# alpc91/SGRL

Hardware: AMD Instinct MI355X
Metric: env-steps/sec (whole node) + SET-actor fwd us/step, 3d_walker mix @8192 envs/GPU (higher is better)
Workload: dtype f64 (dynamics) / f32 (SET actor, obs); 1 GPU; 3D_Walker++ 8 variants x 1024 envs per GPU (config 3), random U(-1,1) actions, auto-reset, SET actor forward on every step, random-init weights; envs_per_gpu=8192, obs_max_len=287, action_max_len=21, replay_gather=none (single rank)

## Files before the change

include/sgrl.h:

```cpp
#ifndef SGRL_H
#define SGRL_H

#include <stdint.h>

#ifdef __cplusplus
extern "C" {
#endif

typedef struct sgrl_engine sgrl_engine;

enum {
  SGRL_OK = 0,
  SGRL_ERR_ARG = -1,
  SGRL_ERR_MODEL = -2,
  SGRL_ERR_HIP = -3,
  SGRL_ERR_LIMIT = -4
};

int sgrl_engine_create(int n_morph, const int32_t* const* ib, const int32_t* ib_len, const double* const* fb,
                       const int32_t* fb_len, const int32_t* morph_count, int obs_max_len, int action_max_len,
                       uint64_t seed, uint32_t env_id_base, int max_episode_steps, sgrl_engine** out);
void sgrl_engine_destroy(sgrl_engine* e);

int sgrl_num_envs(const sgrl_engine* e);
int sgrl_record_stride(const sgrl_engine* e);
int sgrl_lds_bytes(const sgrl_engine* e);
int sgrl_launch_groups(const sgrl_engine* e);
int sgrl_fixed_dim_groups(const sgrl_engine* e);
int sgrl_paired_envs(const sgrl_engine* e);

int sgrl_reset(sgrl_engine* e, float* obs, double* obs64, void* stream);

int sgrl_step(sgrl_engine* e, const float* actions, float* obs, float* reward, uint8_t* done, float* dist,
              uint8_t* truncated, double* obs64, double* reward64, int auto_reset, void* stream);

int sgrl_get_records(sgrl_engine* e, double* rec, int32_t* cnt);
int sgrl_set_records(sgrl_engine* e, const double* rec, const int32_t* cnt);
int sgrl_refresh(sgrl_engine* e, float* obs, double* obs64, void* stream);

int sgrl_time_steps(sgrl_engine* e, const float* actions, float* obs, float* reward, uint8_t* done, int reps,
                    void* stream, float* ms_out);

int sgrl_pack_transitions(const float* obs, int ld_obs, const float* action, int ld_act, const float* next_obs, int ld_next,
                          const float* reward, const float* done_f32, const uint8_t* done_u8, const uint8_t* store,
                          const int64_t* morph_id, float* block, int n_env, int obs_len, int act_len, void* stream);

int sgrl_round_record(const float* reward, const uint8_t* done, uint8_t* done_list, int64_t* ep_steps, float* ep_reward, float* reward_buf,
                      uint8_t* store, float* done_bool, int32_t* all_done, int n_env, int max_episode_steps, void* stream);

typedef struct sgrl_ring {
  float* obs; float* action; float* next_obs; float* reward; float* done;
  int32_t obs_dim, act_dim;
} sgrl_ring;
int sgrl_ingest_rows(const float* block, int n_rows, int obs_len, int act_len, const int64_t* slot, const sgrl_ring* rings,
                     int n_rings, void* stream);
int64_t sgrl_ingest_ws_words(int n_rows);
int sgrl_ingest_block(const float* block, int n_rows, int obs_len, int act_len, const sgrl_ring* rings, int n_rings, int64_t* pos,
                      const int64_t* cap, int64_t* pending, int64_t* slot_ws, void* stream);

const char* sgrl_last_error(void);
const char* sgrl_version(void);

#ifdef __cplusplus
}
#endif
#endif
```

sgrl_amd/_lib.py:

```python
import ctypes
import os
import subprocess

_HERE = os.path.dirname(os.path.abspath(__file__))
LIB_PATH = os.environ.get("SGRL_HIP_LIB", os.path.join(_HERE, "libsgrl_hip.so"))
CSRC = os.path.join(_HERE, "csrc")
SOURCES = ["engine.hip", "set_actor.hip", "train_gemm.hip", "render.hip", "swat_actor.hip", "smp_actor.hip", "replay_sample.hip", "eval_record.hip", "explore_actions.hip", "scene.hip", "mlp_actor.hip", "mlp_train.hip", "mlp_optim.hip", "mlp_batch.hip", "smp_train.hip", "td3_loss.hip", "dropout.hip"]

_lib = None

_i32p = ctypes.POINTER(ctypes.c_int32)
_f64p = ctypes.POINTER(ctypes.c_double)


class SgrlError(RuntimeError):
    pass


HDR_DIM_FIELDS = (1, 2, 3, 4, 5, 6, 7, 8, 9, 16, 18)
LIGHT_NV = 12
ITAB_GLOBAL = set(x for x in os.environ.get("SGRL_BUILD_ITAB_GLOBAL", "humanoid").split(",") if x and x != "none")
PAIR_NV = {"walker": 15, "hopper": 15}


# ... 96 lines not shown
    import torch
    try:
        L = ctypes.CDLL(LIB_PATH)
    except OSError as e:
        raise SgrlError("cannot load %s: %s" % (LIB_PATH, e))
    L.sgrl_last_error.restype = ctypes.c_char_p
    L.sgrl_version.restype = ctypes.c_char_p
    L.sgrl_engine_create.restype = ctypes.c_int
    L.sgrl_engine_create.argtypes = [ctypes.c_int, ctypes.POINTER(_i32p), _i32p, ctypes.POINTER(_f64p), _i32p, _i32p,
                                     ctypes.c_int, ctypes.c_int, ctypes.c_uint64, ctypes.c_uint32, ctypes.c_int,
                                     ctypes.POINTER(ctypes.c_void_p)]
    L.sgrl_engine_destroy.argtypes = [ctypes.c_void_p]
    L.sgrl_engine_destroy.restype = None
    for name in ("sgrl_num_envs", "sgrl_record_stride", "sgrl_lds_bytes", "sgrl_launch_groups", "sgrl_fixed_dim_groups", "sgrl_paired_envs"):
        getattr(L, name).argtypes = [ctypes.c_void_p]
        getattr(L, name).restype = ctypes.c_int
    vp = ctypes.c_void_p
    L.sgrl_reset.argtypes = [vp, vp, vp, vp]
    L.sgrl_step.argtypes = [vp, vp, vp, vp, vp, vp, vp, vp, vp, ctypes.c_int, vp]
    L.sgrl_refresh.argtypes = [vp, vp, vp, vp]
    L.sgrl_get_records.argtypes = [vp, vp, vp]
    L.sgrl_set_records.argtypes = [vp, vp, vp]
    L.sgrl_time_steps.argtypes = [vp, vp, vp, vp, vp, ctypes.c_int, vp, ctypes.POINTER(ctypes.c_float)]
    ci = ctypes.c_int
    L.sgrl_pack_transitions.argtypes = [vp, ci, vp, ci, vp, ci, vp, vp, vp, vp, vp, vp, ci, ci, ci, vp]
    L.sgrl_ingest_rows.argtypes = [vp, ci, ci, ci, vp, vp, ci, vp]
    L.sgrl_ingest_block.argtypes = [vp, ci, ci, ci, vp, ci, vp, vp, vp, vp, vp]
    L.sgrl_round_record.argtypes = [vp, vp, vp, vp, vp, vp, vp, vp, vp, ci, ci, vp]
    L.sgrl_ingest_ws_words.argtypes = [ci]
    L.sgrl_ingest_ws_words.restype = ctypes.c_int64
    _lib = L
    return L


EXPLORE_GAUSS, EXPLORE_UNIFORM = 0, 1


def bind_explore(L):
    if getattr(L, "_explore_bound", False):
        return L
    vp, ci, cf = ctypes.c_void_p, ctypes.c_int, ctypes.c_float
    L.sgrl_explore_actions.argtypes = [vp, ci, vp, ci, vp, ci, ci, ctypes.c_int64, ctypes.c_uint64, ctypes.c_uint64, ci, cf, cf, cf, vp]
    L.sgrl_explore_actions.restype = ci
    L.sgrl_explore_actions_launches.argtypes = []
    L.sgrl_explore_actions_launches.restype = ci
    L.sgrl_explore_last_error.argtypes = []
    L.sgrl_explore_last_error.restype = ctypes.c_char_p
    L._explore_bound = True
    return L


EXPORTS = ["sgrl_engine_create", "sgrl_engine_destroy", "sgrl_num_envs", "sgrl_record_stride", "sgrl_lds_bytes", "sgrl_launch_groups", "sgrl_fixed_dim_groups", "sgrl_paired_envs",
           "sgrl_reset", "sgrl_step", "sgrl_get_records", "sgrl_set_records", "sgrl_refresh", "sgrl_time_steps", "sgrl_pack_transitions", "sgrl_round_record", "sgrl_ingest_rows", "sgrl_ingest_block", "sgrl_ingest_ws_words",
           "sgrl_last_error", "sgrl_version"]


def check(rc, what):
    if rc != 0:
        raise SgrlError("%s failed (%d): %s" % (what, rc, lib().sgrl_last_error().decode()))
```

sgrl_amd/csrc/engine.hip:

```cpp
#include <hip/hip_runtime.h>

#include <algorithm>
#include <cmath>
#include <cstdio>
#include <cstdlib>
#include <cstring>
#include <string>
#include <vector>

#include "engine_kernel.h"
#include "stream_pick.h"

namespace {

thread_local std::string g_err;

int fail(int code, const std::string& msg) {
  g_err = msg;
  return code;
}
#define HIP_TRY(expr)                                                                              \
  do {                                                                                             \
    hipError_t _e = (expr);                                                                        \
    if (_e != hipSuccess)                                                                          \
      return fail(SGRL_ERR_HIP, std::string(#expr) + ": " + hipGetErrorString(_e));                \
  } while (0)

using namespace sgrl_engine_dev;

__global__ __launch_bounds__(64) __attribute__((amdgpu_waves_per_eu(2, 2))) void k_env_step(BatchArgs a, StepOut out) {
  env_step_wave<DimsAny, sgrl::HipWave>(a, out, __builtin_amdgcn_readfirstlane(a.block_env[blockIdx.x]));
}

constexpr int kLightNv = 15;
constexpr int kLightPerCu = 12;
__global__ __launch_bounds__(64) __attribute__((amdgpu_waves_per_eu(3, 3))) void k_env_step_light(BatchArgs a, StepOut out) {
  env_step_wave<DimsAny, sgrl::HipWaveT<kLightNv>>(a, out, __builtin_amdgcn_readfirstlane(a.block_env[blockIdx.x]));
}

__global__ __launch_bounds__(64) void k_env_reset(BatchArgs a, StepOut out) {
  const int env = __builtin_amdgcn_readfirstlane(a.block_env[blockIdx.x]);
  SgrlModelView m; sgrl::Layout o; double* S; int32_t* I;
  setup<DimsAny>(a, env, &m, &o, &S, &I);
  sgrl::HipWave w;
  const sgrl::StepIO io = make_io(a, out, env);
  sgrl::env_reset(w, m, o, S, I, io, true);
}

__global__ __launch_bounds__(64) void k_env_refresh(BatchArgs a, StepOut out) {
  const int env = __builtin_amdgcn_readfirstlane(a.block_env[blockIdx.x]);
  SgrlModelView m; sgrl::Layout o; double* S; int32_t* I;
  setup<DimsAny>(a, env, &m, &o, &S, &I);
  sgrl::HipWave w;
  const sgrl::StepIO io = make_io(a, out, env);
  sgrl::env_refresh(w, m, o, S, I, io);
}

typedef int (*SpecLaunch)(int, int, void*, const void*, const void*);
struct SpecFamily { int waves; int n; SpecLaunch launch; int itab_global; };
struct SpecMember { int family, slot; int dims[12]; };
}
#ifndef SGRL_NO_SPECS
#define SGRL_FAMILY(id, waves, n, itab) extern "C" int sgrl_spec_launch_##id(int, int, void*, const void*, const void*);
#define SGRL_MEMBER(...)
#include "spec_table.inc"
#undef SGRL_FAMILY
#undef SGRL_MEMBER
namespace {
const SpecFamily kFamilies[] = {
#define SGRL_FAMILY(id, waves, n, itab) {waves, n, sgrl_spec_launch_##id, itab},
#define SGRL_MEMBER(...)
#include "spec_table.inc"
#undef SGRL_FAMILY
#undef SGRL_MEMBER
};
const SpecMember kMembers[] = {
#define SGRL_FAMILY(id, waves, n, itab)
#define SGRL_MEMBER(fam, slot, ...) {fam, slot, {__VA_ARGS__}},
#include "spec_table.inc"
#undef SGRL_FAMILY
#undef SGRL_MEMBER
};
constexpr int kNumMembers = (int)(sizeof(kMembers) / sizeof(kMembers[0]));
}
#else
namespace {
const SpecFamily kFamilies[1] = {{0, 0, nullptr, 0}};
const SpecMember kMembers[1] = {{-1, -1, {0}}};
constexpr int kNumMembers = 0;
}
#endif
namespace {
int spec_for(const int32_t* hdr, int waves) {
  static const int fields[11] = {SGRL_H_NBODY, SGRL_H_NJNT, SGRL_H_NQ, SGRL_H_NV, SGRL_H_NU, SGRL_H_NGEOM, SGRL_H_NPAIR,
                                 SGRL_H_INTEGRATOR, SGRL_H_FRAME_SKIP, SGRL_H_MAX_ROWS, SGRL_H_SOLVER};
  for (int k = 0; k < kNumMembers; k++) {
    if (kFamilies[kMembers[k].family].waves != waves) continue;
    bool same = true;
    for (int f = 0; f < 11 && same; f++) same = kMembers[k].dims[f] == hdr[fields[f]];
    if (same) return k;
  }
  return -1;
}
}

struct sgrl_engine {
  int n_morph = 0, n_env = 0, stride = 0, lds_bytes = 0, scratch_stride = 0;
  int obs_max_len = 0, action_max_len = 0;
// ... 188 lines not shown
      for (int g = grp; g < (int)gridDim.x; g += kIngestThreads / kIngestMaxRings) p += w.chunk_hist[g * kIngestMaxRings + ring];
      part[grp][ring] = p;
    }
    __syncthreads();
    if (t < n_rings) {
      long long total = 0;
#pragma unroll
      for (int g = 0; g < kIngestThreads / kIngestMaxRings; g++) total += part[g][t];
      const long long p0 = pos[t];
      w.base[t] = p0;
      pos[t] = (p0 + total) % cap[t];
      pending[t] += total;
    }
    if (t == 0) *w.ticket = 0u;
  }
}
__global__ __launch_bounds__(kIngestThreads) void k_ingest_slots(int n_rows, const long long* __restrict__ cap, long long* ws, long long* __restrict__ slot) {
  __shared__ int keys[kIngestChunk];
  __shared__ int part[8][kIngestMaxRings];
  const IngestWs w = ingest_ws(ws, n_rows);
  const int t = threadIdx.x, c = blockIdx.x, r = c * kIngestChunk + t;
  const int k = r < n_rows ? w.key[r] : -1;
  keys[t] = k;
  {
    const int ring = t & 31, grp = t >> 5;
    int p = 0;
    for (int g = grp; g < c; g += 8) p += w.chunk_hist[g * kIngestMaxRings + ring];
    part[grp][ring] = p;
  }
  __syncthreads();
  long long sl = -1;
  if (k >= 0) {
    int rank = 0;
#pragma unroll
    for (int g = 0; g < 8; g++) rank += part[g][k];
    for (int j = 0; j < t; j++) rank += keys[j] == k ? 1 : 0;
    sl = (w.base[k] + rank) % cap[k];
  }
  if (r < n_rows) slot[r] = sl;
}

extern "C" {

const char* sgrl_last_error(void) { return g_err.c_str(); }
const char* sgrl_version(void) { return "sgrl-hip 0.2.0 (gfx950)"; }
#ifdef SGRL_PHASE_PROF
int sgrl_phase_prof(unsigned long long* host, int n_env, int reset) {
  if (hipDeviceSynchronize() != hipSuccess) return -1;
  if (host && hipMemcpyFromSymbol(host, HIP_SYMBOL(sgrl_engine_dev::g_phase_prof), sizeof(unsigned long long) * 16 * (size_t)n_env) != hipSuccess) return -2;
  if (reset) { static unsigned long long z[16 * 65536]; if (hipMemcpyToSymbol(HIP_SYMBOL(sgrl_engine_dev::g_phase_prof), z, sizeof(z)) != hipSuccess) return -3; }
  return 0;
}
#endif

void sgrl_engine_destroy(sgrl_engine* e) {
  if (!e) return;
  for (auto p : e->d_ib) if (p) (void)hipFree(p);
  for (auto p : e->d_fb) if (p) (void)hipFree(p);
  if (e->d_morphs) (void)hipFree(e->d_morphs);
  if (e->d_env_morph) (void)hipFree(e->d_env_morph);
  if (e->d_block_env) (void)hipFree(e->d_block_env);
  if (e->d_step_env) (void)hipFree(e->d_step_env);
  if (e->d_step_mate) (void)hipFree(e->d_step_mate);
  if (e->d_rec) (void)hipFree(e->d_rec);
  if (e->d_cnt) (void)hipFree(e->d_cnt);
  if (e->d_scratch) (void)hipFree(e->d_scratch);
  if (e->d_cam_dist) (void)hipFree(e->d_cam_dist);
  for (auto& g : e->groups) { if (g.stream) (void)hipStreamDestroy(g.stream); if (g.done) (void)hipEventDestroy(g.done); }
  if (e->fork) (void)hipEventDestroy(e->fork);
  delete e;
}

int sgrl_engine_create(int n_morph, const int32_t* const* ib, const int32_t* ib_len, const double* const* fb,
                       const int32_t* fb_len, const int32_t* morph_count, int obs_max_len, int action_max_len,
                       uint64_t seed, uint32_t env_id_base, int max_episode_steps, sgrl_engine** out) {
  if (!out) return fail(SGRL_ERR_ARG, "out is null");
  *out = nullptr;
  if (n_morph <= 0 || !ib || !ib_len || !fb || !fb_len || !morph_count) return fail(SGRL_ERR_ARG, "null or empty morphology list");
  int ndev = 0;
  (void)hipGetLastError();
  const hipError_t dev_err = hipGetDeviceCount(&ndev);
  if (dev_err != hipSuccess || ndev == 0)
    return fail(SGRL_ERR_HIP, std::string("no HIP device visible: libsgrl_hip.so needs an MI355X (there is no CPU fallback) [") +
                                  hipGetErrorString(dev_err) + ", " + std::to_string(ndev) + " devices]");
  sgrl_engine* e = new sgrl_engine();
  e->n_morph = n_morph;
  e->obs_max_len = obs_max_len;
  e->action_max_len = action_max_len;
  std::vector<int32_t> env_morph;
  std::vector<MorphDev> morphs(n_morph);
  e->d_ib.assign(n_morph, nullptr);
  e->d_fb.assign(n_morph, nullptr);
  int rc = SGRL_OK;
  for (int k = 0; k < n_morph && rc == SGRL_OK; k++) {
    SgrlModelView v;
    if (!ib[k] || !fb[k] || ib_len[k] < SGRL_NHDR || sgrl_model_view(ib[k], fb[k], &v) != 0) { rc = fail(SGRL_ERR_MODEL, "bad magic in model blob " + std::to_string(k)); break; }
    if (v.n_int != ib_len[k] || v.n_f64 != fb_len[k]) { rc = fail(SGRL_ERR_MODEL, "model blob " + std::to_string(k) + " has unexpected length"); break; }
    if (v.nv > 64 || v.nbody > 64 || v.npair > 64) { rc = fail(SGRL_ERR_LIMIT, "morphology exceeds 64 dofs/bodies/pairs"); break; }
    if ((v.nv | 1) > sgrl::kSlabLdy || ib[k][SGRL_H_MAX_ROWS] > sgrl::kSlabRows) { rc = fail(SGRL_ERR_LIMIT, "morphology exceeds the HBM constraint slab (nv <= 46, max_rows <= 256)"); break; }
    e->scratch_stride = std::max(e->scratch_stride, sgrl::slab_doubles(ib[k][SGRL_H_MAX_ROWS], v.nv | 1));
    e->max_geoms = std::max(e->max_geoms, v.ngeom);
    const int L = v.nbody - 1;
    if (41 * L > obs_max_len || 3 * L > action_max_len) { rc = fail(SGRL_ERR_ARG, "obs_max_len/action_max_len too small for morphology " + std::to_string(k)); break; }
    if (morph_count[k] < 0) { rc = fail(SGRL_ERR_ARG, "negative morph_count"); break; }
    sgrl::Layout o;
    sgrl::make_layout(ib[k], &o, v.n_int, SGRL_STAGE_FLOATS ? v.n_f64 : 0);
// ... 364 lines not shown
```

sgrl_amd/csrc/step_body.h:

```cpp
#pragma once

#include <math.h>
#include <stdint.h>

#include "../../include/sgrl_model.h"

#ifdef __HIPCC__
#define SGRL_DEV __device__ __forceinline__
#else
#define SGRL_DEV inline
#endif

namespace sgrl {

constexpr double kMinVal = 1e-15;
constexpr double kMinImp = 0.0001;
constexpr double kMaxImp = 0.9999;
constexpr double kPi = 3.14159265358979323846;
constexpr int kNAMax = 32;
constexpr int kBppMaxIter = 40;
constexpr int kSlabRows = 256;
constexpr int kPivotRows = 64;
constexpr int kPrevRows = 48;
constexpr int kSlabLdy = 47;
// ... 218 lines not shown
  double a[3], b[3], c[3];
  cross3(a, vel, f); cross3(b, vel + 3, f + 3); cross3(c, vel, f + 3);
  r[0] = a[0] + b[0]; r[1] = a[1] + b[1]; r[2] = a[2] + b[2];
  r[3] = c[0]; r[4] = c[1]; r[5] = c[2];
}
SGRL_DEV void ld3(double* r, const double* p) { r[0] = p[0]; r[1] = p[1]; r[2] = p[2]; }
SGRL_DEV void ld6(double* r, const double* p) { r[0] = p[0]; r[1] = p[1]; r[2] = p[2]; r[3] = p[3]; r[4] = p[4]; r[5] = p[5]; }
SGRL_DEV int popcount64(uint64_t x) {
#ifdef __HIPCC__
  return __popcll(x);
#else
  return __builtin_popcountll(x);
#endif
}
SGRL_DEV int clz64(uint64_t x) {
#ifdef __HIPCC__
  return __clzll((long long)x);
#else
  return __builtin_clzll(x);
#endif
}
SGRL_DEV int tri(int i) { return i * (i + 1) / 2; }
SGRL_DEV void tri_decode(int p, int* a_out, int* b_out) {
  int a = (int)((sqrtf(8.0f * (float)p + 1.0f) - 1.0f) * 0.5f);
  a += ((a + 1) * (a + 2) / 2 <= p) ? 1 : 0;
  a -= (a * (a + 1) / 2 > p) ? 1 : 0;
  *a_out = a; *b_out = p - a * (a + 1) / 2;
}
SGRL_DEV bool dof_in_mask(sgrl_itab_t mask2, int d) {
  const uint32_t w = (uint32_t)(d < 32 ? mask2[0] : mask2[1]);
  return (w >> (d & 31)) & 1u;
}

SGRL_DEV double rng_uniform01(uint64_t seed, uint32_t env_id, uint32_t episode, uint32_t stream, uint32_t idx) {
  uint32_t c0 = idx >> 2, c1 = episode, c2 = stream, c3 = (uint32_t)(seed >> 32);
  uint32_t k0 = (uint32_t)seed, k1 = env_id;
  for (int r = 0; r < 10; r++) {
    const uint64_t p0 = (uint64_t)0xD2511F53u * c0, p1 = (uint64_t)0xCD9E8D57u * c2;
    const uint32_t n0 = (uint32_t)(p1 >> 32) ^ c1 ^ k0, n1 = (uint32_t)p1;
    const uint32_t n2 = (uint32_t)(p0 >> 32) ^ c3 ^ k1, n3 = (uint32_t)p0;
    c0 = n0; c1 = n1; c2 = n2; c3 = n3;
    k0 += 0x9E3779B9u; k1 += 0xBB67AE85u;
  }
  const uint32_t lane = idx & 3u;
  const uint32_t x = lane == 0 ? c0 : (lane == 1 ? c1 : (lane == 2 ? c2 : c3));
  return ((double)x + 0.5) * (1.0 / 4294967296.0);
}

#ifdef SGRL_PHASE_PROF
#define SGRL_TICK(id) w.tick(id)
#else
#define SGRL_TICK(id)
#endif

template <class W>
struct Engine {
  W& w;
  SgrlModelView m;
  const Layout& o;
  double* S;
  int32_t* I;
  double* big_scratch = nullptr;
  bool linv = false;

  SGRL_DEV Engine(W& w_, const SgrlModelView& m_, const Layout& o_, double* S_, int32_t* I_)
      : w(w_), m(m_), o(o_), S(S_), I(I_) {}

  SGRL_DEV void fence_view() {
    if (W::kFixedDims) return;
    m.body_parent = w.fenced(m.body_parent); m.body_jntadr = w.fenced(m.body_jntadr);
    m.body_jntnum = w.fenced(m.body_jntnum); m.body_dofadr = w.fenced(m.body_dofadr);
    m.body_dofnum = w.fenced(m.body_dofnum); m.body_limbtype = w.fenced(m.body_limbtype);
    m.jnt_type = w.fenced(m.jnt_type); m.jnt_body = w.fenced(m.jnt_body);
    m.jnt_qposadr = w.fenced(m.jnt_qposadr); m.jnt_dofadr = w.fenced(m.jnt_dofadr);
    m.jnt_limited = w.fenced(m.jnt_limited); m.dof_body = w.fenced(m.dof_body); m.dof_jnt = w.fenced(m.dof_jnt);
    m.dof_parent = w.fenced(m.dof_parent); m.geom_type = w.fenced(m.geom_type);
    m.geom_body = w.fenced(m.geom_body); m.pair_g1 = w.fenced(m.pair_g1); m.pair_g2 = w.fenced(m.pair_g2);
    m.pair_condim = w.fenced(m.pair_condim); m.act_dof = w.fenced(m.act_dof); m.act_slot = w.fenced(m.act_slot);
    m.body_depth = w.fenced(m.body_depth); m.body_path = w.fenced(m.body_path);
    m.body_subend = w.fenced(m.body_subend); m.body_dofmask = w.fenced(m.body_dofmask);
    m.dof_act = w.fenced(m.dof_act);
  }

  SGRL_DEV static void quat_rot(double* r, const double* q, const double* v) {
    double mtx[9];
    quat2mat(mtx, q);
    mat_vec(r, mtx, v);
  }

  SGRL_DEV void kinematics() {
    w.lanes(1, [&](int) {
      double q[4] = {S[o.qpos + 3], S[o.qpos + 4], S[o.qpos + 5], S[o.qpos + 6]};
      quat_normalize(q);
      S[o.qpos + 3] = q[0]; S[o.qpos + 4] = q[1]; S[o.qpos + 5] = q[2]; S[o.qpos + 6] = q[3];
    });
    const int TJ = o.Y, TB = o.Y + 17 * o.nj;
    w.lanes(o.nj, [&](int j) {
      if (m.jnt_type[j] == SGRL_JNT_FREE) return;
      double ja[3], ql[4];
      ld3(ja, m.jnt_axis + 3 * j);
      const int qa = m.jnt_qposadr[j];
      axisangle2quat(ql, ja, S[o.qpos + qa] - m.qpos0[qa]);
      double* t = S + TJ + 17 * j;
      for (int k = 0; k < 4; k++) t[k] = ql[k];
      for (int k = 0; k < 3; k++) { t[4 + k] = ja[k]; t[7 + k] = m.jnt_pos[3 * j + k]; }
    });
// ... 574 lines not shown
        if (hk[r] == key) { f0 = hf[r]; hit = true; }
      }
      if (!hit) {
        for (int k = 0; k < pl; k++) if (I[o.prev_key + k] == key) f0 = S[o.prev_f + k];
        if (pn > pcap) {
          const double* hf = big_scratch + slab_prev_offset(o.maxrows, o.ldy);
          const int32_t* hk = reinterpret_cast<const int32_t*>(hf + o.maxrows);
          for (int k = pcap; k < pn; k++) if (hk[k] == key) f0 = hf[k];
        }
      }
      R.ef[r] = f0;
    });
    SGRL_TICK(6);
    if (linv) {
      if (BIG || !w.trmm_rows(nrow + 1, nv, S + o.L, R.Y, ldy))
      w.lanes(nrow + 1, [&](int r) {
        double* Yr = R.Y + r * ldy;
        for (int d = nv - 1; d >= 0; d--) {
          const double* Ld = S + o.L + tri(d);
          double s0 = 0, s1 = 0, s2 = 0, s3 = 0;
          int c = 0;
          for (; c + 4 <= d + 1; c += 4) {
            const double a0 = Ld[c], a1 = Ld[c + 1], a2 = Ld[c + 2], a3 = Ld[c + 3];
            const double b0 = Yr[c], b1 = Yr[c + 1], b2 = Yr[c + 2], b3 = Yr[c + 3];
            s0 += a0 * b0; s1 += a1 * b1; s2 += a2 * b2; s3 += a3 * b3;
          }
          for (; c <= d; c++) s0 += Ld[c] * Yr[c];
          Yr[d] = (s0 + s1) + (s2 + s3);
        }
      });
    } else {
      w.trsm_lower_rows(nrow + 1, nv, S + o.L, S + o.dinv, R.Y, ldy);
    }
    SGRL_TICK(9);
    w.lanes(nrow > nv ? nrow : nv, [&](int r) {
      if (r < nrow) {
        const double* Yr = R.Y + r * ldy;
        const double* ys = R.Y + nrow * ldy;
        double q0 = 0, q1 = 0, t0 = 0, t1 = 0;
        int d = 0;
        for (; d + 2 <= nv; d += 2) {
          const double y0 = Yr[d], y1 = Yr[d + 1];
          q0 += y0 * y0; q1 += y1 * y1; t0 += y0 * ys[d]; t1 += y1 * ys[d + 1];
        }
        for (; d < nv; d++) { q0 += Yr[d] * Yr[d]; t0 += Yr[d] * ys[d]; }
        const double Rr = R.eR[r];
        R.eidg[r] = 1.0 / ((q0 + q1) + Rr);
        R.eb[r] = (t0 + t1) - R.earef[r];
      }
      if (r < nv) S[o.vpgs + r] = 0;
    });
  }

  template <bool SMALL, bool CLDS>
  SGRL_DEV bool lcp_block_pivot(const Rows& R, int n, double thresh, int* iters_out) {
    double* const wvp = R.earef;
    double* const xwp = SMALL ? S + o.prev_f : S + o.Y;
    const int nv = o.nv, ldy = o.ldy;
    uint64_t F = w.ballot(n, [&](int i) { return R.ef[i] > 0.0; });
    int patience = 3, best = n + 1;
    for (int iter = 0; iter < kBppMaxIter; iter++) {
      w.fence_lane();
      const int nf = popcount64(F);
      double* const C = CLDS ? S + o.dead : R.C;
      w.lanes(n, [&](int i) {
        if ((F >> i) & 1ull) {
          const int pos = popcount64(F & ((1ull << i) - 1ull));
          R.flist[pos] = i;
          xwp[pos] = -R.eb[i];
        }
      });
      if (!w.aff_rows(nf, nv, R.Y, ldy, R.flist, R.eR, C))
      w.lanes(nf * (nf + 1) / 2, [&](int p) {
        int i, j;
        tri_decode(p, &i, &j);
        const int fi = R.flist[i], fj = R.flist[j];
        const double* yi = R.Y + fi * ldy;
        const double* yj = R.Y + fj * ldy;
        double s0 = 0, s1 = 0, s2 = 0, s3 = 0;
        int d = 0;
        for (; d + 4 <= nv; d += 4) {
          const double a0 = yi[d], a1 = yi[d + 1], a2 = yi[d + 2], a3 = yi[d + 3];
          const double b0 = yj[d], b1 = yj[d + 1], b2 = yj[d + 2], b3 = yj[d + 3];
          s0 += a0 * b0; s1 += a1 * b1; s2 += a2 * b2; s3 += a3 * b3;
        }
        for (; d < nv; d++) s0 += yi[d] * yj[d];
        double a = (s0 + s1) + (s2 + s3);
        if (i == j) a += R.eR[fi];
        C[p] = a;
      });
      SGRL_TICK(12);
      if (SMALL && w.chol_inv_packed(nf, C, kMinVal)) {
        w.lanes(nf, [&](int i) {
          double z = 0;
          for (int c = 0; c <= i; c++) z += C[i * (i + 1) / 2 + c] * xwp[c];
          wvp[i] = z;
        });
        w.lanes(nf, [&](int k) {
          double x = 0;
          for (int i = k; i < nf; i++) x += C[i * (i + 1) / 2 + k] * wvp[i];
          xwp[k] = x;
        });
      } else {
        for (int j = 0; j < nf - 1; j++) {
          double pj = C[j * (j + 1) / 2 + j];
          if (pj < kMinVal) pj = kMinVal;
          const double wj = 1.0 / pj;
          const int sdim = nf - j - 1;
          w.lanes(sdim * (sdim + 1) / 2, [&](int p) {
            int a, b;
            tri_decode(p, &a, &b);
            const int i = j + 1 + a, k = j + 1 + b;
            C[i * (i + 1) / 2 + k] -= C[i * (i + 1) / 2 + j] * C[k * (k + 1) / 2 + j] * wj;
          });
        }
        w.lanes(nf, [&](int j) {
          double pj = C[j * (j + 1) / 2 + j];
          if (pj < kMinVal) pj = kMinVal;
          wvp[j] = 1.0 / pj;
        });
        for (int j = 0; j < nf; j++) {
          const double zj = xwp[j] * wvp[j];
          w.lanes_from(j + 1, nf, [&](int i) { xwp[i] -= C[i * (i + 1) / 2 + j] * zj; });
        }
        w.lanes(nf, [&](int i) { xwp[i] *= wvp[i]; });
        for (int j = nf - 1; j > 0; j--) {
          const double xj = xwp[j];
          w.lanes(j, [&](int k) { xwp[k] -= C[j * (j + 1) / 2 + k] * wvp[k] * xj; });
        }
      }
      SGRL_TICK(13);
      w.lanes(nv, [&](int d) {
        double u0 = 0, u1 = 0;
        int k = 0;
        for (; k + 2 <= nf; k += 2) { u0 += R.Y[R.flist[k] * ldy + d] * xwp[k]; u1 += R.Y[R.flist[k + 1] * ldy + d] * xwp[k + 1]; }
        if (k < nf) u0 += R.Y[R.flist[k] * ldy + d] * xwp[k];
        S[o.vpgs + d] = u0 + u1;
      });
      const uint64_t V = w.ballot(n, [&](int i) {
        if ((F >> i) & 1ull) return xwp[popcount64(F & ((1ull << i) - 1ull))] < -thresh * R.eidg[i];
        const double* yi = R.Y + i * ldy;
        double y0 = R.eb[i], y1 = 0, y2 = 0, y3 = 0;
        int d = 0;
        for (; d + 4 <= nv; d += 4) {
          y0 += yi[d] * S[o.vpgs + d]; y1 += yi[d + 1] * S[o.vpgs + d + 1];
// ... 438 lines not shown
```

sgrl_amd/csrc/wave_half.h:

```cpp
#pragma once
#include <stdint.h>

#include "step_body.h"

namespace sgrl {

template <int NVCAP, class P>
struct HalfWaveT : P {
  static_assert(NVCAP <= 16, "the register solvers of a half wave keep one matrix row per lane of ONE 16-lane DPP row");
  using P::lane;
  static constexpr int kLanes = 32;

  template <class F> SGRL_DEV void lanes(int n, F f) {
    for (int i = lane; i < n; i += kLanes) f(i);
    P::sync();
  }
  template <class F> SGRL_DEV void lanes_from(int lo, int hi, F f) {
    for (int i = lo + lane; i < hi; i += kLanes) f(i);
    P::sync();
  }
  template <class F> SGRL_DEV double sum(int n, F f) {
    double p = 0.0;
    for (int i = lane; i < n; i += kLanes) p += f(i);
    return P::half_sum(p);
  }
  template <class F> SGRL_DEV double maxabs(int n, F f) {
    double p = 0.0;
    for (int i = lane; i < n; i += kLanes) p = fmax(p, fabs(f(i)));
    return P::half_max(p);
  }
  template <class F> SGRL_DEV uint64_t ballot(int n, F f) {
    uint64_t m = P::half_ballot(lane < n ? (bool)f(lane) : false);
    if (n > kLanes) m |= (uint64_t)P::half_ballot(lane + kLanes < n ? (bool)f(lane + kLanes) : false) << 32;
    return m;
  }

  template <int NMAX>
  SGRL_DEV void chol_inv_reg(int n, double* Pm, double minval) {
    const bool act = lane < n;
    const int li = act ? lane : 0;
    double* rowp = Pm + li * (li + 1) / 2;
    double a[NMAX + 1];
#pragma unroll
    for (int k = 0; k < NMAX; k++) a[k + 1] = rowp[k < li ? k : li];
    double mydj = 0.0;
#pragma unroll
    for (int j = 0; j < NMAX; j++) {
      if (j < n) {
        const double c = a[j + 1];
        double pj = P::bcast16(c, j);
        pj = pj < minval ? minval : pj;
        const double dj = inv_sqrt(pj);
        const double l = c * dj;
        mydj = lane == j ? dj : mydj;
        const double lm = lane > j ? l * dj : 0.0;
        a[j] = lane == j ? 1.0 : 0.0;
#pragma unroll
        for (int c2 = 0; c2 <= j; c2++) a[c2] -= lm * P::bcast16(a[c2], j);
#pragma unroll
        for (int k = j + 1; k < NMAX; k++) a[k + 1] -= l * P::bcast16(l, k);
      }
    }
    if (act) {
#pragma unroll
      for (int k = NMAX - 1; k >= 0; k--) rowp[k < li ? k : li] = a[k] * mydj;
    }
    P::sync();
  }
  SGRL_DEV bool chol_inv_packed(int n, double* Pm, double minval) {
    if (NVCAP >= 9 && n <= 9) chol_inv_reg<9>(n, Pm, minval);
    else if (NVCAP >= 12 && n <= 12) chol_inv_reg<12>(n, Pm, minval);
    else if (NVCAP >= 15 && n <= 15) chol_inv_reg<15>(n, Pm, minval);
    else return false;
    return true;
  }

  template <int NMAX>
  SGRL_DEV void trmm_rows_reg(int nrhs, int n, const double* T, double* Y, int ldy) {
    constexpr int NH = (NMAX + 1) / 2;
    const int h = lane & 1;
    for (int r0 = 0; r0 < nrhs; r0 += kLanes / 2) {
      const int r = r0 + (lane >> 1);
      const bool act = r < nrhs;
      double* y = Y + (act ? r : nrhs - 1) * ldy;
      double jr[NH];
#pragma unroll
      for (int u = 0; u < NH; u++) {
        const int c = 2 * u + h;
        const double v = y[c < n ? c : n - 1];
        jr[u] = c < n ? v : 0.0;
      }
#pragma unroll
      for (int d = (NMAX - 1) | 1; d >= 1; d -= 2) {
        if (d - 1 < n) {
          const double* Td = T + d * (d + 1) / 2 + h;
          const double* Te = T + (d - 1) * d / 2 + h;
          double s0 = 0.0, s1 = 0.0, e0 = 0.0, e1 = 0.0;
#pragma unroll
          for (int u = 0; u < NH; u++) {
            if (2 * u + 1 <= d) {
              const double td = Td[2 * u], te = Te[2 * u];
              const double tem = (2 * u + 1 <= d - 1) ? te : (h == 0 ? te : 0.0);
              if (u & 1) { s1 += td * jr[u]; e1 += tem * jr[u]; } else { s0 += td * jr[u]; e0 += tem * jr[u]; }
            }
          }
          double sd = s0 + s1, se = e0 + e1;
          sd += P::xor1(sd);
          se += P::xor1(se);
          if (act) { if (h == 0) y[d - 1] = se; else if (d < n) y[d] = sd; }
        }
      }
    }
    P::sync();
  }
  SGRL_DEV bool trmm_rows(int nrhs, int n, const double* T, double* Y, int ldy) {
#ifdef SGRL_NO_TRMM
    return false;
#endif
    if (NVCAP >= 9 && n <= 9) trmm_rows_reg<9>(nrhs, n, T, Y, ldy);
    else if (NVCAP >= 12 && n <= 12) trmm_rows_reg<12>(nrhs, n, T, Y, ldy);
    else if (NVCAP >= 15 && n <= 15) trmm_rows_reg<15>(nrhs, n, T, Y, ldy);
    else return false;
    return true;
  }
  SGRL_DEV bool aff_rows(int, int, const double*, int, const int32_t*, const double*, double*) { return false; }
// ... 68 lines not shown
```

sgrl_amd/csrc/wave_hip.h:

```cpp
#pragma once
#include <hip/hip_runtime.h>

#include "../../include/sgrl_model.h"

namespace sgrl {

template <int CTRL>
__device__ __forceinline__ double dpp_move(double x) {
  int lo = __double2loint(x), hi = __double2hiint(x);
  lo = __builtin_amdgcn_update_dpp(0, lo, CTRL, 0xF, 0xF, false);
  hi = __builtin_amdgcn_update_dpp(0, hi, CTRL, 0xF, 0xF, false);
  return __hiloint2double(hi, lo);
}
__device__ __forceinline__ double read_lane(double x, int l) {
  const int lo = __builtin_amdgcn_readlane(__double2loint(x), l);
  const int hi = __builtin_amdgcn_readlane(__double2hiint(x), l);
  return __hiloint2double(hi, lo);
}
__device__ __forceinline__ double wave_sum(double x) {
  x += dpp_move<0xB1>(x);
  x += dpp_move<0x4E>(x);
  x += dpp_move<0x141>(x);
  x += dpp_move<0x140>(x);
  return (read_lane(x, 0) + read_lane(x, 16)) + (read_lane(x, 32) + read_lane(x, 48));
// ... 138 lines not shown
        change = fmax(change, fabs(df) / ir);
      }
      __syncthreads();
      if (change < thresh) { it++; break; }
    }
    if (dofl) v[lane] = vv;
    __syncthreads();
    return it;
  }
  template <int NMAX>
  __device__ __forceinline__ void chol_inv_reg(int n, double* P, double minval) {
    const bool act = lane < n;
    const int li = act ? lane : 0;
    double* rowp = P + li * (li + 1) / 2;
    double a[NMAX + 1];
#pragma unroll
    for (int k = 0; k < NMAX; k++) a[k + 1] = rowp[k < li ? k : li];
    double mydj = 0.0;
#pragma unroll
    for (int j = 0; j < NMAX; j++) {
      if (j < n) {
        const double c = a[j + 1];
        double pj = read_lane(c, j);
        pj = pj < minval ? minval : pj;
        const double dj = rsqrt(pj);
        const double l = c * dj;
        mydj = lane == j ? dj : mydj;
        const double lm = lane > j ? l * dj : 0.0;
        a[j] = lane == j ? 1.0 : 0.0;
#pragma unroll
        for (int c2 = 0; c2 <= j; c2++) a[c2] -= lm * read_lane(a[c2], j);
#pragma unroll
        for (int k = j + 1; k < NMAX; k++) a[k + 1] -= l * read_lane(l, k);
      }
    }
    if (act) {
#pragma unroll
      for (int k = NMAX - 1; k >= 0; k--) rowp[k < li ? k : li] = a[k] * mydj;
    }
    __syncthreads();
  }
  __device__ __forceinline__ bool chol_inv_packed(int n_in, double* P, double minval) {
    const int n = __builtin_amdgcn_readfirstlane(n_in);
    if (NVCAP >= 9 && n <= 9) chol_inv_reg<9>(n, P, minval);
    else if (NVCAP >= 12 && n <= 12) chol_inv_reg<12>(n, P, minval);
    else if (NVCAP >= 15 && n <= 15) chol_inv_reg<15>(n, P, minval);
    else if (NVCAP >= 18 && n <= 18) chol_inv_reg<18>(n, P, minval);
    else if (NVCAP >= 21 && n <= 21) chol_inv_reg<21>(n, P, minval);
    else if (NVCAP >= 24 && n <= 24) chol_inv_reg<24>(n, P, minval);
    else return false;
    return true;
  }
  template <int NMAX>
  __device__ __forceinline__ void trmm_rows_reg(int nrhs, int n, const double* T, double* Y, int ldy) {
    constexpr int NH = (NMAX + 1) / 2;
    const int h = lane & 1;
    for (int r0 = 0; r0 < nrhs; r0 += 32) {
      const int r = r0 + (lane >> 1);
      const bool act = r < nrhs;
      double* y = Y + (act ? r : nrhs - 1) * ldy;
      double jr[NH];
#pragma unroll
      for (int u = 0; u < NH; u++) {
        const int c = 2 * u + h;
        const double v = y[c < n ? c : n - 1];
        jr[u] = c < n ? v : 0.0;
      }
#pragma unroll
      for (int d = (NMAX - 1) | 1; d >= 1; d -= 2) {
        if (d - 1 < n) {
          const double* Td = T + d * (d + 1) / 2 + h;
          const double* Te = T + (d - 1) * d / 2 + h;
          double s0 = 0.0, s1 = 0.0, e0 = 0.0, e1 = 0.0;
#pragma unroll
          for (int u = 0; u < NH; u++) {
            if (2 * u + 1 <= d) {
              const double td = Td[2 * u], te = Te[2 * u];
              const double tem = (2 * u + 1 <= d - 1) ? te : (h == 0 ? te : 0.0);
              if (u & 1) { s1 += td * jr[u]; e1 += tem * jr[u]; } else { s0 += td * jr[u]; e0 += tem * jr[u]; }
            }
          }
          double sd = s0 + s1, se = e0 + e1;
          sd += dpp_move<0xB1>(sd);
          se += dpp_move<0xB1>(se);
          if (act) { if (h == 0) y[d - 1] = se; else if (d < n) y[d] = sd; }
        }
      }
    }
    __syncthreads();
  }
  __device__ __forceinline__ void trmm_rows_mfma(int nrhs, int n, const double* T, double* Y, int ldy) {
    const int lo = lane & 15, hi = lane >> 4;
    const int ksteps = (n + 3) >> 2;
    for (int r0 = 0; r0 < nrhs; r0 += 16) {
      const int r = r0 + lo;
      const bool rv = r < nrhs;
      const double* yr = Y + (rv ? r : 0) * ldy;
      double b[6];
#pragma unroll
      for (int s = 0; s < 6; s++) {
        const int c = 4 * s + hi;
        const double v = yr[c < n ? c : 0];
        b[s] = (rv && c < n) ? v : 0.0;
      }
#pragma unroll
      for (int dt = 0; dt < 2; dt++) {
// ... 221 lines not shown
```

Measured before the change: 2.035 million env-steps/s.

## Fuse Cholesky factorization with forward/back solve instead of explicit inverse

Measured after the change: 2.079 million env-steps/s (median of 6 runs). 2.2% higher.

```diff
diff --git a/include/sgrl.h b/include/sgrl.h
--- a/include/sgrl.h
+++ b/include/sgrl.h
@@ -58,6 +58,9 @@
 int sgrl_ingest_block(const float* block, int n_rows, int obs_len, int act_len, const sgrl_ring* rings, int n_rings, int64_t* pos,
                       const int64_t* cap, int64_t* pending, int64_t* slot_ws, void* stream);
 
+#define SGRL_DEBUG_CHOL_LD 352
+int sgrl_debug_chol_solve(int flags, const int32_t* n, const double* C, const double* rhs, double* C_out, double* x_out, int32_t* ok);
+
 const char* sgrl_last_error(void);
 const char* sgrl_version(void);
 
diff --git a/sgrl_amd/_lib.py b/sgrl_amd/_lib.py
--- a/sgrl_amd/_lib.py
+++ b/sgrl_amd/_lib.py
@@ -172,7 +172,7 @@
 
 EXPORTS = ["sgrl_engine_create", "sgrl_engine_destroy", "sgrl_num_envs", "sgrl_record_stride", "sgrl_lds_bytes", "sgrl_launch_groups", "sgrl_fixed_dim_groups", "sgrl_paired_envs",
            "sgrl_reset", "sgrl_step", "sgrl_get_records", "sgrl_set_records", "sgrl_refresh", "sgrl_time_steps", "sgrl_pack_transitions", "sgrl_round_record", "sgrl_ingest_rows", "sgrl_ingest_block", "sgrl_ingest_ws_words",
-           "sgrl_last_error", "sgrl_version"]
+           "sgrl_debug_chol_solve", "sgrl_last_error", "sgrl_version"]
 
 
 def check(rc, what):
diff --git a/sgrl_amd/csrc/engine.hip b/sgrl_amd/csrc/engine.hip
--- a/sgrl_amd/csrc/engine.hip
+++ b/sgrl_amd/csrc/engine.hip
@@ -54,6 +54,50 @@
   sgrl::HipWave w;
   const sgrl::StepIO io = make_io(a, out, env);
   sgrl::env_refresh(w, m, o, S, I, io);
+}
+
+template <class Wv>
+__device__ __forceinline__ void debug_chol_solve(Wv& w, int n, double* C, double* x, double* wv, bool inverse, int32_t* ok) {
+  bool done;
+  if (!inverse) {
+    done = w.chol_solve_packed(n, C, x, sgrl::kMinVal);
+  } else {
+    done = w.chol_inv_packed(n, C, sgrl::kMinVal);
+    if (done) {
+      w.lanes(n, [&](int i) {
+        double z = 0;
+        for (int c = 0; c <= i; c++) z += C[i * (i + 1) / 2 + c] * x[c];
+        wv[i] = z;
+      });
+      w.lanes(n, [&](int k) {
+        double s = 0;
+        for (int i = k; i < n; i++) s += C[i * (i + 1) / 2 + k] * wv[i];
+        x[k] = s;
+      });
+    }
+  }
+  if (w.lane == 0) *ok = done ? 1 : 0;
+}
+__global__ __launch_bounds__(64) void k_debug_chol_solve(int flags, const int32_t* n, const double* C, const double* rhs, double* C_out,
+                                                         double* x_out, int32_t* ok) {
+  constexpr int LD = SGRL_DEBUG_CHOL_LD;
+  __shared__ double sC[2 * LD], sx[64], swv[64];
+  const int t = threadIdx.x;
+  for (int i = t; i < 2 * LD; i += 64) sC[i] = C[i];
+  sx[t] = rhs[t];
+  swv[t] = 0.0;
+  __syncthreads();
+  if (flags & 1) {
+    sgrl::HalfWaveT<15, sgrl::HipHalfPrim<sgrl::DimsAny>> w;
+    const int h = w.half;
+    debug_chol_solve(w, n[h], sC + h * LD, sx + h * 32, swv + h * 32, (flags & 2) != 0, ok + h);
+  } else {
+    sgrl::HipWave w;
+    debug_chol_solve(w, n[0], sC, sx, swv, (flags & 2) != 0, ok);
+  }
+  __syncthreads();
+  for (int i = t; i < 2 * LD; i += 64) C_out[i] = sC[i];
+  x_out[t] = sx[t];
 }
 
 typedef int (*SpecLaunch)(int, int, void*, const void*, const void*);
@@ -348,6 +392,34 @@
   return 0;
 }
 #endif
+
+int sgrl_debug_chol_solve(int flags, const int32_t* n, const double* C, const double* rhs, double* C_out, double* x_out, int32_t* ok) {
+  constexpr int LD = SGRL_DEBUG_CHOL_LD;
+  if (!n || !C || !rhs || !C_out || !x_out || !ok) return fail(SGRL_ERR_ARG, "sgrl_debug_chol_solve: null pointer");
+  for (int p = 0; p < ((flags & 1) ? 2 : 1); p++)
+    if (n[p] < 0 || n[p] * (n[p] + 1) / 2 > LD) return fail(SGRL_ERR_ARG, "sgrl_debug_chol_solve: n out of range");
+  const size_t bytes = sizeof(double) * (4 * LD + 128) + sizeof(int32_t) * 4;
+  char* d = nullptr;
+  HIP_TRY(hipMalloc((void**)&d, bytes));
+  double* dC = (double*)d; double* dCo = dC + 2 * LD; double* dr = dCo + 2 * LD; double* dx = dr + 64;
+  int32_t* dn = (int32_t*)(dx + 64); int32_t* dok = dn + 2;
+  const int32_t n2[2] = {n[0], (flags & 1) ? n[1] : 0};
+  hipError_t e = hipMemset(d, 0, bytes);
+  if (e == hipSuccess) e = hipMemcpy(dC, C, sizeof(double) * 2 * LD, hipMemcpyHostToDevice);
+  if (e == hipSuccess) e = hipMemcpy(dr, rhs, sizeof(double) * 64, hipMemcpyHostToDevice);
+  if (e == hipSuccess) e = hipMemcpy(dn, n2, sizeof(n2), hipMemcpyHostToDevice);
+  if (e == hipSuccess) {
+    k_debug_chol_solve<<<1, 64>>>(flags, dn, dC, dr, dCo, dx, dok);
+    e = hipGetLastError();
+  }
+  if (e == hipSuccess) e = hipDeviceSynchronize();
+  if (e == hipSuccess) e = hipMemcpy(C_out, dCo, sizeof(double) * 2 * LD, hipMemcpyDeviceToHost);
+  if (e == hipSuccess) e = hipMemcpy(x_out, dx, sizeof(double) * 64, hipMemcpyDeviceToHost);
+  if (e == hipSuccess) e = hipMemcpy(ok, dok, sizeof(int32_t) * 2, hipMemcpyDeviceToHost);
+  (void)hipFree(d);
+  if (e != hipSuccess) return fail(SGRL_ERR_HIP, std::string("sgrl_debug_chol_solve: ") + hipGetErrorString(e));
+  return SGRL_OK;
+}
 
 void sgrl_engine_destroy(sgrl_engine* e) {
   if (!e) return;
diff --git a/sgrl_amd/csrc/step_body.h b/sgrl_amd/csrc/step_body.h
--- a/sgrl_amd/csrc/step_body.h
+++ b/sgrl_amd/csrc/step_body.h
@@ -294,6 +294,14 @@
 #else
 #define SGRL_TICK(id)
 #endif
+
+template <class T> T& ref_of();
+template <class Wv, class = void>
+struct HasCholSolve { static constexpr bool value = false; };
+template <class Wv>
+struct HasCholSolve<Wv, decltype((void)ref_of<Wv>().chol_solve_packed(0, ref_of<double*>(), ref_of<double*>(), 0.0))> {
+  static constexpr bool value = true;
+};
 
 template <class W>
 struct Engine {
@@ -974,6 +982,12 @@
     });
   }
 
+  template <bool SMALL>
+  SGRL_DEV bool chol_solve_small(int nf, double* C, double* x) {
+    if constexpr (SMALL && HasCholSolve<W>::value) return w.chol_solve_packed(nf, C, x, kMinVal);
+    else return false;
+  }
+
   template <bool SMALL, bool CLDS>
   SGRL_DEV bool lcp_block_pivot(const Rows& R, int n, double thresh, int* iters_out) {
     double* const wvp = R.earef;
@@ -992,7 +1006,7 @@
           xwp[pos] = -R.eb[i];
         }
       });
-      if (!w.aff_rows(nf, nv, R.Y, ldy, R.flist, R.eR, C))
+      if (nf > 0 && !w.aff_rows(nf, nv, R.Y, ldy, R.flist, R.eR, C))
       w.lanes(nf * (nf + 1) / 2, [&](int p) {
         int i, j;
         tri_decode(p, &i, &j);
@@ -1012,7 +1026,9 @@
         C[p] = a;
       });
       SGRL_TICK(12);
-      if (SMALL && w.chol_inv_packed(nf, C, kMinVal)) {
+      if (nf == 0) {
+      } else if (chol_solve_small<SMALL>(nf, C, xwp)) {
+      } else if (SMALL && !HasCholSolve<W>::value && w.chol_inv_packed(nf, C, kMinVal)) {
         w.lanes(nf, [&](int i) {
           double z = 0;
           for (int c = 0; c <= i; c++) z += C[i * (i + 1) / 2 + c] * xwp[c];
diff --git a/sgrl_amd/csrc/wave_half.h b/sgrl_amd/csrc/wave_half.h
--- a/sgrl_amd/csrc/wave_half.h
+++ b/sgrl_amd/csrc/wave_half.h
@@ -71,6 +71,59 @@
     if (NVCAP >= 9 && n <= 9) chol_inv_reg<9>(n, Pm, minval);
     else if (NVCAP >= 12 && n <= 12) chol_inv_reg<12>(n, Pm, minval);
     else if (NVCAP >= 15 && n <= 15) chol_inv_reg<15>(n, Pm, minval);
+    else return false;
+    return true;
+  }
+
+  template <int NMAX>
+  SGRL_DEV void chol_solve_reg(int n, double* Pm, double* x, double minval) {
+    const bool act = lane < n;
+    const int li = act ? lane : 0;
+    double* rowp = Pm + li * (li + 1) / 2;
+    double a[NMAX];
+#pragma unroll
+    for (int k = 0; k < NMAX; k++) a[k] = rowp[k < li ? k : li];
+    double r = x[li];
+#pragma unroll
+    for (int j = 0; j < NMAX; j++) {
+      if (j < n) {
+        const double c = a[j];
+        double pj = P::bcast16(c, j);
+        pj = pj < minval ? minval : pj;
+        const double dj = inv_sqrt(pj);
+        const double l = c * dj;
+        const double lb = lane > j ? l : 0.0;
+        const double zj = P::bcast16(r, j) * dj;
+        r = lane == j ? zj * dj : r - lb * zj;
+        a[j] = lb * dj;
+#pragma unroll
+        for (int k = j + 1; k < NMAX; k++) a[k] -= l * P::bcast16(l, k);
+      }
+    }
+    if (act) {
+#pragma unroll
+      for (int k = NMAX - 1; k >= 0; k--) rowp[k < li ? k : li] = a[k];
+    }
+    P::sync();
+    const int nl = n > 0 ? n - 1 : 0;
+#pragma unroll
+    for (int j = 1; j < NMAX; j++) {
+      const int jj = j < nl ? j : nl;
+      a[j] = Pm[jj * (jj + 1) / 2 + (lane < jj ? lane : jj)];
+    }
+#pragma unroll
+    for (int j = NMAX - 1; j >= 1; j--) {
+      if (j < n) r -= a[j] * P::bcast16(r, j);
+    }
+    if (act) x[lane] = r;
+    P::sync();
+  }
+  SGRL_DEV bool chol_solve_packed(int n, double* Pm, double* x, double minval) {
+    if (n <= 3) chol_solve_reg<3>(n, Pm, x, minval);
+    else if (n <= 6) chol_solve_reg<6>(n, Pm, x, minval);
+    else if (NVCAP >= 9 && n <= 9) chol_solve_reg<9>(n, Pm, x, minval);
+    else if (NVCAP >= 12 && n <= 12) chol_solve_reg<12>(n, Pm, x, minval);
+    else if (NVCAP >= 15 && n <= 15) chol_solve_reg<15>(n, Pm, x, minval);
     else return false;
     return true;
   }
diff --git a/sgrl_amd/csrc/wave_hip.h b/sgrl_amd/csrc/wave_hip.h
--- a/sgrl_amd/csrc/wave_hip.h
+++ b/sgrl_amd/csrc/wave_hip.h
@@ -214,6 +214,62 @@
     return true;
   }
   template <int NMAX>
+  __device__ __forceinline__ void chol_solve_reg(int n, double* P, double* x, double minval) {
+    const bool act = lane < n;
+    const int li = act ? lane : 0;
+    double* rowp = P + li * (li + 1) / 2;
+    double a[NMAX];
+#pragma unroll
+    for (int k = 0; k < NMAX; k++) a[k] = rowp[k < li ? k : li];
+    double r = x[li];
+#pragma unroll
+    for (int j = 0; j < NMAX; j++) {
+      if (j < n) {
+        const double c = a[j];
+        double pj = read_lane(c, j);
+        pj = pj < minval ? minval : pj;
+        const double dj = rsqrt(pj);
+        const double l = c * dj;
+        const double lb = lane > j ? l : 0.0;
+        const double zj = read_lane(r, j) * dj;
+        r = lane == j ? zj * dj : r - lb * zj;
+        a[j] = lb * dj;
+#pragma unroll
+        for (int k = j + 1; k < NMAX; k++) a[k] -= l * read_lane(l, k);
+      }
+    }
+    if (act) {
+#pragma unroll
+      for (int k = NMAX - 1; k >= 0; k--) rowp[k < li ? k : li] = a[k];
+    }
+    __syncthreads();
+    const int nl = n > 0 ? n - 1 : 0;
+#pragma unroll
+    for (int j = 1; j < NMAX; j++) {
+      const int jj = j < nl ? j : nl;
+      a[j] = P[jj * (jj + 1) / 2 + (lane < jj ? lane : jj)];
+    }
+#pragma unroll
+    for (int j = NMAX - 1; j >= 1; j--) {
+      if (j < n) r -= a[j] * read_lane(r, j);
+    }
+    if (act) x[lane] = r;
+    __syncthreads();
+  }
+  __device__ __forceinline__ bool chol_solve_packed(int n_in, double* P, double* x, double minval) {
+    const int n = __builtin_amdgcn_readfirstlane(n_in);
+    if (n <= 3) chol_solve_reg<3>(n, P, x, minval);
+    else if (n <= 6) chol_solve_reg<6>(n, P, x, minval);
+    else if (NVCAP >= 9 && n <= 9) chol_solve_reg<9>(n, P, x, minval);
+    else if (NVCAP >= 12 && n <= 12) chol_solve_reg<12>(n, P, x, minval);
+    else if (NVCAP >= 15 && n <= 15) chol_solve_reg<15>(n, P, x, minval);
+    else if (NVCAP >= 18 && n <= 18) chol_solve_reg<18>(n, P, x, minval);
+    else if (NVCAP >= 21 && n <= 21) chol_solve_reg<21>(n, P, x, minval);
+    else if (NVCAP >= 24 && n <= 24) chol_solve_reg<24>(n, P, x, minval);
+    else return false;
+    return true;
+  }
+  template <int NMAX>
   __device__ __forceinline__ void trmm_rows_reg(int nrhs, int n, const double* T, double* Y, int ldy) {
     constexpr int NH = (NMAX + 1) / 2;
     const int h = lane & 1;
```
